# vlongle/pixie

Measured on AMD Instinct MI355X. Metric: voxels/s (128^3 U-Net fwd) + MPM particle-steps/s, higher is better.
Workload: dtype f32 (operands split fp16 hi+lo, 3 f16 MFMAs/product, fp32 accumulate); 1 GPU; 128^3x64 feature grid -> SegmentationUNet+RegressionUNet forward (+argmax/one-hot combine), 1 scene per GPU per step; grid=128, feature_channels=64, parallelism=scene-parallel x1, executor=c+hip_graph

## Files before the change

### include/pixie_hip.h

```cpp
#ifndef PIXIE_HIP_H
#define PIXIE_HIP_H

#include <stdint.h>

#ifdef __cplusplus
extern "C" {
#endif

const char* pixie_last_error(void);
const char* pixie_build_arch(void);

typedef struct pixie_mpm pixie_mpm;

int pixie_mpm_create(pixie_mpm** out, int n_particles, int n_grid, double grid_lim);
int pixie_mpm_destroy(pixie_mpm* h);
int pixie_mpm_regrid(pixie_mpm* h, int n_grid, double grid_lim, void* stream);

int pixie_mpm_set_field(pixie_mpm* h, const char* name, const void* d_src, int64_t count, void* stream);
int pixie_mpm_get_field(pixie_mpm* h, const char* name, void* d_dst, int64_t count, void* stream);
int pixie_mpm_fill_field(pixie_mpm* h, const char* name, double value, void* stream);

int pixie_mpm_set_scalar(pixie_mpm* h, const char* key, double value);
int pixie_mpm_get_scalar(pixie_mpm* h, const char* key, double* value);

// ... 133 lines not shown

int pixie_combine_class_ids(const int32_t* d_seg_pred, int num_classes, const float* d_cont, int64_t spatial, float* d_combined,
                            void* stream);

typedef struct pixie_unet pixie_unet;
typedef struct pixie_unet_config {
    int32_t feature_channels, cond_dim, model_channels, num_res_blocks;
    int32_t n_channel_mult; int32_t channel_mult[8];
    int32_t n_attention_resolutions; int32_t attention_resolutions[8];
    int32_t grid_size;
    int32_t out_channels;
    int32_t precision;
} pixie_unet_config;

int pixie_unet_create(pixie_unet** out, const pixie_unet_config* cfg);
int pixie_unet_destroy(pixie_unet* h);
int pixie_unet_param_count(const pixie_unet* h);
int pixie_unet_param_info(const pixie_unet* h, int index, const char** key, int64_t* numel, int32_t* ndim, int64_t shape[5]);
int pixie_unet_set_param(pixie_unet* h, const char* key, const float* d_values, int64_t numel);
int64_t pixie_unet_workspace_bytes(pixie_unet* h, int d, int hh, int w);
int pixie_unet_forward(pixie_unet* h, const float* d_feat, const float* d_proj0, int d, int hh, int w, float* d_out,
                       void* d_workspace, int64_t workspace_bytes, void* stream);
int pixie_unet_set_option(pixie_unet* h, const char* key, int value);

typedef struct pixie_field_desc {
    const float* d_pred;
    const uint8_t* d_mask;
    const float* d_axis_x; const float* d_axis_y; const float* d_axis_z;
    int32_t n_classes, d, h, w;
    double min_spacing;
    double density_min, density_max, E_min, E_max, nu_min, nu_max;
} pixie_field_desc;
int pixie_field_to_particles(const pixie_field_desc* field, const float* d_pos, int n, int k, double nn_distance_threshold,
                             int weighted, int default_material, int default_part_label, float* d_density, float* d_E,
                             float* d_nu, int32_t* d_material, int32_t* d_part_label, float* d_conf, float* d_nearest,
                             void* d_scratch, void* stream);

int pixie_unscale_prediction(const float* d_pred, int channels, int64_t spatial, double density_min, double density_max,
                             double E_min, double E_max, double nu_min, double nu_max, float* d_out, void* stream);
int64_t pixie_field_points_scratch_bytes(const pixie_field_desc* field);
int pixie_field_points(const pixie_field_desc* field, int64_t capacity, float* d_xyz , float* d_density, float* d_E,
                       float* d_nu, int32_t* d_material, float* d_conf, int64_t* d_count, void* d_scratch, void* stream);

int pixie_dbscan_roots(const float* d_pos_sorted, const int32_t* d_orig_index, const int32_t* d_cell_start, int n, int nx, int ny, int nz,
                       const double lo[3], double cell_size, double eps, int min_samples, int32_t* d_core_scratch,
                       int32_t* d_parent_scratch, int32_t* d_root, void* stream);
// ... 51 lines not shown
```

### pixie_amd/_lib.py

```python
from __future__ import annotations

import ctypes as C
import os

_HERE = os.path.dirname(os.path.abspath(__file__))
LIB_PATH = os.path.join(_HERE, "libpixie_hip.so")
DIAG_LIB_PATH = os.path.join(_HERE, "libpixie_hip_diag.so")


class PixieHipError(RuntimeError):
    pass


class BCDesc(C.Structure):
    _fields_ = [("type", C.c_int32), ("surface_type", C.c_int32), ("reset", C.c_int32), ("pad_", C.c_int32),
                ("point", C.c_double * 3), ("size", C.c_double * 3), ("velocity", C.c_double * 3),
                ("normal", C.c_double * 3), ("start_time", C.c_double), ("end_time", C.c_double),
                ("friction", C.c_double)]


class PModDesc(C.Structure):
    _fields_ = [("type", C.c_int32), ("pad_", C.c_int32),
                ("point", C.c_double * 3), ("size", C.c_double * 3), ("force", C.c_double * 3),
                ("velocity", C.c_double * 3), ("normal", C.c_double * 3), ("h1", C.c_double * 3),
# ... 100 lines not shown
    "pixie_conv_subpixel_bytes": (_I64, [_I, _I]),
    "pixie_conv_pack_weights_subpixel": (_I, [_VP, _VP, _I, _I, _VP]),
    "pixie_conv3d_forward": (_I, [C.POINTER(ConvDesc), _VP]),
    "pixie_conv_stats_floats": (_I64, [C.POINTER(ConvDesc)]),
    "pixie_conv_workspace_bytes": (_I64, [C.POINTER(ConvDesc)]),
    "pixie_stats_finalize": (_I, [_VP, C.POINTER(ConvDesc), _VP, _VP]),
    "pixie_stats_norm_finalize": (_I, [_VP, C.POINTER(ConvDesc), _VP, _VP, C.POINTER(ConvDesc), _VP, _I, _I64, _I, _I, _D, _VP, _VP, _VP, _VP, _VP]),
    "pixie_channel_stats": (_I, [_VP, _I, _I64, _VP, _VP, _VP]),
    "pixie_tensor_amax": (_I, [_VP, _I64, _VP, _VP]),
    "pixie_channel_sums": (_I, [_VP, _I, _I64, _VP, _VP]),
    "pixie_norm_finalize": (_I, [_VP, _I, _I64, _I, _I, _D, _VP, _VP, _VP, _VP, _VP]),
    "pixie_attention_forward": (_I, [_VP, _VP, _I, _I, _VP]),
    "pixie_channel_affine": (_I, [_VP, _VP, _VP, _VP, _I, _I64, _VP]),
    "pixie_projector_conv0": (_I, [_VP, _I64, _I, _I, C.POINTER(_VP), C.POINTER(_VP), C.POINTER(_VP), _I, _VP]),
    "pixie_conv_skip_foldable": (_I, [C.POINTER(ConvDesc)]),
    "pixie_unet_create": (_I, [C.POINTER(_VP), C.POINTER(UNetConfigC)]),
    "pixie_unet_destroy": (_I, [_VP]),
    "pixie_unet_param_count": (_I, [_VP]),
    "pixie_unet_param_info": (_I, [_VP, _I, C.POINTER(_S), C.POINTER(_I64), C.POINTER(C.c_int32), C.POINTER(_I64)]),
    "pixie_unet_set_param": (_I, [_VP, _S, _VP, _I64]),
    "pixie_unet_workspace_bytes": (_I64, [_VP, _I, _I, _I]),
    "pixie_unet_set_option": (_I, [_VP, _S, _I]),
    "pixie_unet_forward": (_I, [_VP, _VP, _VP, _I, _I, _I, _VP, _VP, _I64, _VP]),
    "pixie_combine_class_ids": (_I, [_VP, _I, _VP, _I64, _VP, _VP]),
    "pixie_combine_predictions": (_I, [_VP, _I, _VP, _I64, _VP, _VP, _VP]),
    "pixie_voxel_grid_to_ncdhw": (_I, [_VP, _I, _I, _I, _I, _VP, _VP]),
    "pixie_unscale_prediction": (_I, [_VP, _I, _I64, _D, _D, _D, _D, _D, _D, _VP, _VP]),
    "pixie_field_points_scratch_bytes": (_I64, [C.POINTER(FieldDesc)]),
    "pixie_field_points": (_I, [C.POINTER(FieldDesc), _I64, _VP, _VP, _VP, _VP, _VP, _VP, _VP, _VP, _VP]),
    "pixie_fill_densify": (_I, [_VP, _VP, _VP, _I, _I, _D, _VP, _VP, _VP]),
    "pixie_fill_dense_cells": (_I, [_VP, _VP, _I, _D, _D, _I, _VP, _I64, _VP, C.c_uint32, _VP]),
    "pixie_fill_internal_cells": (_I, [_VP, _VP, _I, _D, _I, _I, _I, _D, _VP, _I64, _VP, C.c_uint32, _VP]),
    "pixie_particle_volume": (_I, [_VP, _I, _I, _D, _VP, _VP, _VP]),
    "pixie_nearest_particle": (_I, [_VP, _I, _VP, _I, _VP, _VP]),
    "pixie_dbscan_roots": (_I, [_VP, _VP, _VP, _I, _I, _I, _I, C.POINTER(_D), _D, _D, _I, _VP, _VP, _VP, _VP]),
    "pixie_raster_workspace_bytes": (_I64, [_I, _I, _I, _I64]),
    "pixie_raster_forward": (_I, [C.POINTER(RasterDesc), C.POINTER(_I64), _VP]),
    "pixie_sh_to_rgb": (_I, [_VP, _I64, _I, _I, _VP, C.POINTER(C.c_float), _VP, _I64, _VP, _VP]),
    "pixie_field_to_particles": (_I, [C.POINTER(FieldDesc), _VP, _I, _I, _D, _I, _I, _I, _VP, _VP, _VP, _VP, _VP, _VP, _VP, _VP, _VP]),
}

DIAG_SIGNATURES = {
    "pixie_mpm_phase": (_I, [_VP, _I, _D, _VP]),
    "pixie_mpm_kernel_times": (_I, [_VP, C.POINTER(_D), C.POINTER(_D), C.POINTER(_I64)]),
    "pixie_conv_kernel_variant": (C.c_int, [C.POINTER(ConvDesc), C.POINTER(C.c_int)]),
    "pixie_conv_tile_geometry": (C.c_int, [C.POINTER(ConvDesc), C.POINTER(C.c_int32)]),
# ... 41 lines not shown
```

### pixie_amd/csrc/unet_exec.hip

```cpp
#include <hip/hip_runtime.h>

#include <algorithm>
#include <cmath>
#include <cstdlib>
#include <cstring>
#include <map>
#include <memory>
#include <stdexcept>
#include <string>
#include <tuple>
#include <unordered_map>
#include <vector>

#include "../../include/pixie_hip.h"
#include "common.h"

namespace pixie {
int channel_stats_prezeroed(const float* d_x, int channels, int64_t spatial, double* d_sums, uint32_t* d_amax, hipStream_t st);
int norm_finalize_cat(const double* d_sums0, int c0, const double* d_sums1, int c1, int64_t spatial, int mode, int groups, double eps,
                      const float* d_weight, const float* d_bias, float* d_a, float* d_b, hipStream_t st);
namespace {

enum { ACT_NONE = 0, ACT_LEAKY = 1, ACT_SILU = 2 };
enum Kind { CONV_IN, RES, DOWN, ATTN, UP };
// ... 161 lines not shown
            used_[off] = bytes;
            if (off + bytes > peak) peak = off + bytes;
            return off;
        }
        fail("pixie_unet_forward: the workspace is too small (%lld bytes; ask pixie_unet_workspace_bytes for this grid size)", (long long)capacity);
    }
    void release(int64_t off) {
        auto u = used_.find(off);
        if (u == used_.end()) return;
        int64_t size = u->second;
        used_.erase(u);
        auto next = free_.lower_bound(off);
        if (next != free_.end() && off + size == next->first) { size += next->second; next = free_.erase(next); }
        if (next != free_.begin()) {
            auto prev = std::prev(next);
            if (prev->first + prev->second == off) { prev->second += size; return; }
        }
        free_[off] = size;
    }
    template <class T> T* ptr(int64_t off) const { return reinterpret_cast<T*>(base + off); }
};

struct Exec;
struct Tens {
    Exec* ex = nullptr;
    float* p = nullptr;
    int64_t off = -1;
    int c = 0, d = 0, h = 0, w = 0;
    int64_t sums_off = -1;
    bool has_sums = false;
    double* sums = nullptr;
    int64_t partials_off = -1;
    pixie_conv_desc pdesc;
    uint32_t* slot = nullptr;
    int64_t spatial() const { return (int64_t)d * h * w; }
    ~Tens();
};
using TP = std::shared_ptr<Tens>;

struct Packed { void* d = nullptr; uint64_t version = ~0ull; };
struct Sized { int64_t bytes; int slots; int64_t zsum_doubles; };
struct Bound { float wmax = 0, bmax = 0; uint64_t wver = ~0ull, bver = ~0ull; };

}
}

using namespace pixie;

struct pixie_unet {
    Cfg cfg;
    Plan plan;
    std::vector<Param> params;
    std::unordered_map<std::string, int> index;
    std::unordered_map<std::string, Packed> packed32, packed16;
    std::unordered_map<std::string, Bound> bounds;
    uint32_t* d_bound_slots = nullptr;
    std::vector<uint32_t> h_bound_slots;
    std::map<std::tuple<int, int, int, bool>, Sized> sized;
    bool fuse_stats = true, split_k = true, fold_skip = true, subpixel = true;
    bool split_stats = true;
    struct Replay { const float* feat; const float* proj0; float* out; void* ws; int d; uint64_t epoch; hipGraph_t graph; hipGraphExec_t exec; };
    bool use_graph = false;
    uint64_t epoch = 0;
    std::vector<Replay> replays;
    static constexpr size_t kMaxReplays = 4;
    void drop_replay(size_t i) {
        (void)hipGraphExecDestroy(replays[i].exec);
        (void)hipGraphDestroy(replays[i].graph);
        replays.erase(replays.begin() + (long)i);
    }

    const Param& param(const std::string& key) const {
        auto it = index.find(key);
        if (it == index.end()) fail("pixie_unet: no parameter named '%s'", key.c_str());
        return params[it->second];
    }
};

namespace pixie {
namespace {

struct Exec {
    pixie_unet* net = nullptr;
    Arena arena;
    bool dry = false;
    void* stream = nullptr;
    uint32_t* slots = nullptr;
    int slot_next = 0, slot_cap = 0;
// ... 49 lines not shown
        if (dry) return nullptr;
        Packed& e = net->packed32[key];
        if (e.version != p.version) {
            const int cout = (int)p.shape[0], cin = (int)p.shape[1], k = (int)p.shape[2];
            int64_t taps = 1;
            for (size_t i = 2; i < p.shape.size(); ++i) taps *= p.shape[i];
            const int64_t nb = taps * cin * pixie_conv_cout_padded(cout) * (int64_t)sizeof(float);
            if (!e.d && hipMalloc(&e.d, (size_t)nb) != hipSuccess) fail("pixie_unet: hipMalloc of %lld bytes failed", (long long)nb);
            if (!p.d) fail("pixie_unet_forward: parameter '%s.weight' was never set", key.c_str());
            ok(pixie_conv_pack_weights(p.d, static_cast<float*>(e.d), cout, cin, k, stream), "pixie_conv_pack_weights");
            e.version = p.version;
        }
        return static_cast<const float*>(e.d);
    }
    float norm_bound(const std::string& key, int64_t count) {
        if (dry) return 1.0f;
        const Bound& b = net->bounds[key];
        return (float)(std::sqrt((double)count) * (double)b.wmax + (double)b.bmax + 1e-30);
    }

    void stats(const TP& t) {
        if (t->has_sums || t->partials_off >= 0) return;
        t->has_sums = true;
        if (!dry && zsum_next + 2 * t->c > zsum_cap) fail("pixie_unet_forward: out of statistics space (internal sizing error)");
        t->sums = dry ? nullptr : zsums + zsum_next;
        zsum_next += 2 * t->c;
        t->slot = new_slot();
        if (!dry) ok(channel_stats_prezeroed(t->p, t->c, t->spatial(), t->sums, t->slot, as_stream(stream)), "pixie_channel_stats");
    }
    struct AB { std::shared_ptr<Scratch> mem; float* a; float* b; };
    AB norm_finalize(const std::vector<TP>& parts, int64_t spatial, int mode, int groups, const float* w, const float* b) {
        for (auto& t : parts) stats(t);
        const Tens* t0 = parts[0].get();
        const Tens* t1 = parts.size() > 1 ? parts[1].get() : nullptr;
        const int c0 = t0->c, c1 = t1 ? t1->c : 0, c = c0 + c1;
        AB r;
        const int cpad = (c + 63) / 64 * 64;
        r.mem = std::make_shared<Scratch>(this, (int64_t)(cpad + c) * sizeof(float));
        r.a = r.mem->as<float>();
        r.b = r.a + cpad;
        const bool p0 = t0->partials_off >= 0, p1 = t1 && t1->partials_off >= 0;
        if (p0 || p1) {
            pixie_conv_desc d0 = t0->pdesc;
            if (!p0) { std::memset(&d0, 0, sizeof d0); d0.c_out = c0; }
            if (!dry) ok(pixie_stats_norm_finalize(p0 ? arena.ptr<float>(t0->partials_off) : nullptr, &d0, t0->sums,
                                                   p1 ? arena.ptr<float>(t1->partials_off) : nullptr, p1 ? &t1->pdesc : nullptr, t1 ? t1->sums : nullptr,
// ... 140 lines not shown
        const int64_t spatial = x->spatial();
        AB pro = norm_finalize({x}, spatial, 1, 32, P(p + ".norm.weight"), P(p + ".norm.bias"));
        ConvOpt o; o.pro = &pro; o.bound = norm_bound(p + ".norm", spatial * (c / 32));
        TP qkv = conv({x}, p + ".qkv", 3 * c, 1, o);
        TP att = make(c, x->d, x->h, x->w);
        if (!dry) ok(pixie_attention_forward(qkv->p, att->p, c, (int)spatial, stream), "pixie_attention_forward");
        qkv.reset();
        ConvOpt o2; o2.residual = x;
        return conv({att}, p + ".proj_out", c, 1, o2);
    }
    TP block(const Blk& b, const std::vector<TP>& parts, const Tens* up_to) {
        if (b.kind == RES) return res(b, parts);
        const TP& x = parts[0];
        if (b.kind == ATTN) return attn(b, x);
        if (b.kind == DOWN) { ConvOpt o; o.stride = 2; return conv({x}, b.prefix + ".op", b.cout, 3, o); }
        if (b.kind == UP) {
            ConvOpt o; o.upsample = true;
            if (up_to) { o.out_d = up_to->d; o.out_h = up_to->h; o.out_w = up_to->w; }
            return conv({x}, b.prefix + ".conv", b.cout, 3, o);
        }
        fail("pixie_unet: unexpected block kind");
    }

    TP forward(const float* d_feat, const float* d_proj0, int D, int H, int W, float* d_out) {
        const Cfg& c = net->cfg;
        const int64_t spatial = (int64_t)D * H * W;
        TP x;
        AB pro_in; const AB* pro_in_p = nullptr;
        int act_in = ACT_NONE; float bound_in = 0.0f;
        if (c.has_projector()) {
            const std::string q = "projector.net.";
            const int hid = c.projector_hidden();
            if (!hid) {
                const int g = std::max(c.cond_dim / 2, 1);
                x = conv({external(d_feat, c.feature_channels, D, H, W)}, q + "0", c.cond_dim, 1, ConvOpt{});
                pro_in = norm_finalize({x}, spatial, 1, g, P(q + "1.weight"), P(q + "1.bias"));
                act_in = ACT_SILU;
                bound_in = norm_bound(q + "1", spatial * (c.cond_dim / g));
            } else {
                if (d_proj0) x = external(d_proj0, hid, D, H, W);
                else x = conv({external(d_feat, c.feature_channels, D, H, W)}, q + "0", hid, 1, ConvOpt{});
                AB pro = norm_finalize({x}, spatial, 1, 32, P(q + "1.weight"), P(q + "1.bias"));
                ConvOpt o; o.pro = &pro; o.act = ACT_SILU; o.bound = norm_bound(q + "1", spatial * (hid / 32));
                x = conv({x}, q + "3", hid, 3, o);
                AB pro2 = norm_finalize({x}, spatial, 1, 32, P(q + "4.weight"), P(q + "4.bias"));
                ConvOpt o2; o2.pro = &pro2; o2.act = ACT_SILU; o2.bound = norm_bound(q + "4", spatial * (hid / 32));
                x = conv({x}, q + "6", c.cond_dim, 1, o2);
                pro_in = norm_finalize({x}, spatial, 1, 32, P(q + "7.weight"), P(q + "7.bias"));
                bound_in = norm_bound(q + "7", spatial * std::max(c.cond_dim / 32, 1));
            }
            pro_in_p = &pro_in;
        } else {
            x = external(d_feat, c.feature_channels, D, H, W);
        }
        const Plan& plan = net->plan;
        std::vector<TP> hs;
        const Blk& first = plan.in_blocks[0][0];
        ConvOpt of; of.pro = pro_in_p; of.act = act_in; of.bound = bound_in;
        TP h = conv({x}, first.prefix, first.cout, 3, of);
        x.reset();
        pro_in = AB{};
        hs.push_back(h);
        for (size_t i = 1; i < plan.in_blocks.size(); ++i) {
            for (const Blk& b : plan.in_blocks[i]) h = block(b, {h}, nullptr);
            hs.push_back(h);
        }
        for (const Blk& b : plan.middle) h = block(b, {h}, nullptr);
        for (auto& seq : plan.out_blocks) {
            TP skip = hs.back(); hs.pop_back();
            if (skip->d != h->d || skip->h != h->h || skip->w != h->w) fail("pixie_unet_forward: skip tensor and decoder tensor differ in size");
            std::vector<TP> parts{h, skip};
            h.reset(); skip.reset();
            for (const Blk& b : seq) {
                TP nh = block(b, parts, (b.kind == UP && !hs.empty()) ? hs.back().get() : nullptr);
                parts.clear();
                parts.push_back(nh);
            }
            h = parts[0];
        }
        AB pro = norm_finalize({h}, h->spatial(), 0, 1, nullptr, nullptr);
        ConvOpt oo; oo.pro = &pro; oo.affine_store = "unet.out.0"; oo.act = ACT_LEAKY; oo.bound = norm_bound("unet.out.0", h->spatial());
        oo.out_ptr = d_out;
        return conv({h}, "unet.out.2", c.out_channels, 3, oo);
    }
};

Tens::~Tens() {
    if (!ex) return;
    if (off >= 0) ex->arena.release(off);
    if (sums_off >= 0) ex->arena.release(sums_off);
    if (partials_off >= 0) ex->arena.release(partials_off);
}

void refresh_bounds(pixie_unet* net, void* stream) {
    std::vector<std::pair<std::string, int>> todo;
    int n_norm = 0;
    for (const Param& p : net->params) {
        if (!p.norm || p.key.size() < 7 || p.key.compare(p.key.size() - 7, 7, ".weight") != 0) continue;
        const std::string key = p.key.substr(0, p.key.size() - 7);
        const Param& pb = net->param(key + ".bias");
        Bound& b = net->bounds[key];
        if (b.wver != p.version || b.bver != pb.version) todo.push_back({key, 2 * n_norm});
        ++n_norm;
    }
    if (todo.empty()) return;
    const size_t bytes = (size_t)2 * n_norm * sizeof(uint32_t);
// ... 25 lines not shown
    if (i < n16) p[i] = make_uint4(0u, 0u, 0u, 0u);
}

constexpr int64_t kSlotAlign = 256;
int64_t slot_region_bytes(int n_slots) { return ((int64_t)n_slots * 4 + kSlotAlign - 1) / kSlotAlign * kSlotAlign; }
int64_t zsum_region_bytes(int64_t n_doubles) { return (n_doubles * 8 + kSlotAlign - 1) / kSlotAlign * kSlotAlign; }

Sized size_pass(pixie_unet* net, int D, int H, int W, bool from_proj0) {
    auto key = std::make_tuple(D, H, W, from_proj0);
    auto it = net->sized.find(key);
    if (it != net->sized.end()) return it->second;
    Exec ex;
    ex.net = net; ex.dry = true; ex.stream = nullptr;
    ex.arena.reset(reinterpret_cast<char*>(0x10000000), (int64_t)1 << 50);
    {
        const float* fake = reinterpret_cast<const float*>(0x100);
        TP out = ex.forward(from_proj0 ? nullptr : fake, from_proj0 ? fake : nullptr, D, H, W, reinterpret_cast<float*>(0x100));
    }
    Sized r{ex.arena.peak + slot_region_bytes(ex.slot_next) + zsum_region_bytes(ex.zsum_next), ex.slot_next, ex.zsum_next};
    net->sized[key] = r;
    return r;
}

template <class F> int guarded(F f) {
    try { return f(); }
    catch (const std::exception& e) { return set_error("%s", e.what()); }
}

}
}

extern "C" int pixie_unet_create(pixie_unet** out, const pixie_unet_config* c) {
    PX_REQUIRE(out && c, "pixie_unet_create: null argument");
    PX_REQUIRE(c->n_channel_mult >= 1 && c->n_channel_mult <= 8 && c->n_attention_resolutions >= 0 && c->n_attention_resolutions <= 8,
               "pixie_unet_create: channel_mult needs 1..8 entries, attention_resolutions 0..8");
    PX_REQUIRE(c->feature_channels > 0 && c->cond_dim > 0 && c->model_channels > 0 && c->num_res_blocks > 0 && c->grid_size > 0 && c->out_channels > 0,
               "pixie_unet_create: non-positive size");
    PX_REQUIRE(c->precision == 0 || c->precision == 1, "pixie_unet_create: precision is 0 (f16x3) or 1 (exact fp32)");
    return guarded([&] {
        std::unique_ptr<pixie_unet> n(new pixie_unet);
        n->cfg.feature_channels = c->feature_channels; n->cfg.cond_dim = c->cond_dim; n->cfg.model_channels = c->model_channels;
        n->cfg.num_res_blocks = c->num_res_blocks; n->cfg.grid_size = c->grid_size; n->cfg.out_channels = c->out_channels;
        n->cfg.precision = c->precision;
        n->cfg.mult.assign(c->channel_mult, c->channel_mult + c->n_channel_mult);
        n->cfg.attn.assign(c->attention_resolutions, c->attention_resolutions + c->n_attention_resolutions);
        n->plan = build_plan(n->cfg);
        n->params = param_table(n->cfg, n->plan);
        for (size_t i = 0; i < n->params.size(); ++i) n->index[n->params[i].key] = (int)i;
        const char* fs = getenv("PIXIE_FUSE_STATS"); n->fuse_stats = !(fs && fs[0] == '0');
        const char* sk = getenv("PIXIE_CONV_SPLIT_K"); n->split_k = !(sk && sk[0] == '0');
        const char* fk = getenv("PIXIE_FOLD_SKIP"); n->fold_skip = !(fk && fk[0] == '0');
        const char* ss = getenv("PIXIE_SPLIT_STATS"); n->split_stats = !(ss && ss[0] == '0');
        const char* sx = getenv("PIXIE_CONV_SUBPIXEL"); n->subpixel = !(sx && sx[0] == '0');
        *out = n.release();
        return 0;
    });
}

extern "C" int pixie_unet_destroy(pixie_unet* h) {
    if (!h) return 0;
    for (auto& kv : h->packed16) if (kv.second.d) (void)hipFree(kv.second.d);
    for (auto& kv : h->packed32) if (kv.second.d) (void)hipFree(kv.second.d);
    if (h->d_bound_slots) (void)hipFree(h->d_bound_slots);
    while (!h->replays.empty()) h->drop_replay(0);
    delete h;
    return 0;
}

extern "C" int pixie_unet_param_count(const pixie_unet* h) { return h ? (int)h->params.size() : 0; }

extern "C" int pixie_unet_param_info(const pixie_unet* h, int i, const char** key, int64_t* numel, int32_t* ndim, int64_t shape[5]) {
    PX_REQUIRE(h && i >= 0 && i < (int)h->params.size(), "pixie_unet_param_info: index out of range");
    const Param& p = h->params[i];
    if (key) *key = p.key.c_str();
    if (numel) *numel = p.numel;
    if (ndim) *ndim = (int32_t)p.shape.size();
    if (shape) for (size_t k = 0; k < p.shape.size() && k < 5; ++k) shape[k] = p.shape[k];
    return 0;
}

extern "C" int pixie_unet_set_param(pixie_unet* h, const char* key, const float* d_values, int64_t numel) {
    PX_REQUIRE(h && key && d_values, "pixie_unet_set_param: null argument");
    auto it = h->index.find(key);
    PX_REQUIRE(it != h->index.end(), "pixie_unet_set_param: unexpected key '%s' (the reference's load_state_dict(strict=True) raises here too)", key);
    Param& p = h->params[it->second];
    PX_REQUIRE(numel == p.numel, "pixie_unet_set_param: '%s' has %lld elements, got %lld", key, (long long)p.numel, (long long)numel);
    p.d = d_values;
// ... 6 lines not shown
    if (!h || d <= 0 || hh <= 0 || w <= 0) { set_error("pixie_unet_workspace_bytes: bad argument"); return -1; }
    int64_t bytes = -1;
    const int rc = guarded([&] {
        bytes = size_pass(h, d, hh, w, false).bytes;
        if (h->cfg.projector_hidden() > 0) bytes = std::max(bytes, size_pass(h, d, hh, w, true).bytes);
        return 0;
    });
    return rc == 0 ? bytes : -1;
}

extern "C" int pixie_unet_forward(pixie_unet* h, const float* d_feat, const float* d_proj0, int d, int hh, int w, float* d_out,
                                  void* d_workspace, int64_t workspace_bytes, void* stream) {
    PX_REQUIRE(h && d_out && d_workspace && (d_feat || d_proj0), "pixie_unet_forward: null argument");
    PX_REQUIRE(d == h->cfg.grid_size && hh == d && w == d,
               "pixie_unet_forward: the network was built for a %d^3 grid (its LayerNorm parameters have that shape), got %d x %d x %d", h->cfg.grid_size, d, hh, w);
    PX_REQUIRE(!d_proj0 || h->cfg.projector_hidden() > 0, "pixie_unet_forward: d_proj0 needs the hidden-128 projector (feature_channels > cond_dim)");
    PX_REQUIRE(d_feat || (d_proj0 && h->cfg.has_projector()), "pixie_unet_forward: d_feat is null");
    return guarded([&] {
        const auto sized = size_pass(h, d, hh, w, d_proj0 != nullptr);
        if (workspace_bytes < sized.bytes)
            fail("pixie_unet_forward: workspace of %lld bytes, this grid needs %lld (pixie_unet_workspace_bytes)", (long long)workspace_bytes, (long long)sized.bytes);
        auto launch_all = [&] {
            Exec ex;
            ex.net = h; ex.dry = false; ex.stream = stream;
            const int64_t slot_bytes = slot_region_bytes(sized.slots), head_bytes = slot_bytes + zsum_region_bytes(sized.zsum_doubles);
            ex.slots = static_cast<uint32_t*>(d_workspace);
            ex.slot_cap = sized.slots;
            ex.zsums = reinterpret_cast<double*>(static_cast<char*>(d_workspace) + slot_bytes);
            ex.zsum_cap = sized.zsum_doubles;
            hipLaunchKernelGGL(zero_head_kernel, dim3((unsigned)((head_bytes / 16 + 255) / 256)), dim3(256), 0, as_stream(stream),
                               static_cast<uint4*>(d_workspace), head_bytes / 16);
            if (hipGetLastError() != hipSuccess) fail("pixie_unet_forward: clearing the workspace head failed");
            ex.arena.reset(static_cast<char*>(d_workspace) + head_bytes, workspace_bytes - head_bytes);
            TP out = ex.forward(d_feat, d_proj0, d, hh, w, d_out);
        };
        if (h->use_graph) {
            for (size_t i = 0; i < h->replays.size(); ++i) {
                const pixie_unet::Replay& r = h->replays[i];
                if (r.feat != d_feat || r.proj0 != d_proj0 || r.out != d_out || r.ws != d_workspace || r.d != d) continue;
                if (r.epoch != h->epoch) { h->drop_replay(i); break; }
                if (hipGraphLaunch(r.exec, as_stream(stream)) != hipSuccess) fail("pixie_unet_forward: hipGraphLaunch failed: %s", hipGetErrorString(hipGetLastError()));
                if (i + 1 != h->replays.size()) std::rotate(h->replays.begin() + (long)i, h->replays.begin() + (long)i + 1, h->replays.end());
                return 0;
            }
        }
        if (h->use_graph && as_stream(stream) == nullptr)
            fail("pixie_unet_forward: option \"graph\" needs a non-default stream (the legacy stream cannot be captured); pass a created stream or set graph = 0");
        refresh_bounds(h, stream);
        launch_all();
        if (h->use_graph) {
            hipStream_t st = as_stream(stream);
            if (hipStreamBeginCapture(st, hipStreamCaptureModeThreadLocal) != hipSuccess)
                fail("pixie_unet_forward: cannot capture on this stream (graph replay needs a non-default stream): %s", hipGetErrorString(hipGetLastError()));
            hipGraph_t graph = nullptr;
            try { launch_all(); }
            catch (...) { (void)hipStreamEndCapture(st, &graph); if (graph) (void)hipGraphDestroy(graph); throw; }
            if (hipStreamEndCapture(st, &graph) != hipSuccess || !graph) fail("pixie_unet_forward: hipStreamEndCapture failed: %s", hipGetErrorString(hipGetLastError()));
            hipGraphExec_t exec = nullptr;
            if (hipGraphInstantiate(&exec, graph, nullptr, nullptr, 0) != hipSuccess) { (void)hipGraphDestroy(graph); fail("pixie_unet_forward: hipGraphInstantiate failed"); }
            if (h->replays.size() >= pixie_unet::kMaxReplays) h->drop_replay(0);
            h->replays.push_back(pixie_unet::Replay{d_feat, d_proj0, d_out, d_workspace, d, h->epoch, graph, exec});
        }
        return 0;
    });
}

extern "C" int pixie_unet_set_option(pixie_unet* h, const char* key, int value) {
    PX_REQUIRE(h && key, "pixie_unet_set_option: null argument");
    const std::string k(key);
    if (k == "graph") {
        h->use_graph = value != 0;
        if (!h->use_graph) while (!h->replays.empty()) h->drop_replay(0);
        return 0;
    }
    return set_error("pixie_unet_set_option: unknown key '%s' (known: graph)", key);
}
```

### pixie_amd/unet.py

```python
from __future__ import annotations

import ctypes as C
import math
import os
import warnings
import weakref
from typing import Dict, List, Optional, Sequence, Tuple

import torch
import torch.nn as nn

from . import _lib
from ._lib import ConvDesc, check
from .unet_plan import Block, UNetConfig, UNetPlan, build_plan, param_shapes, is_norm_key

ACT_NONE, ACT_LEAKY, ACT_SILU = 0, 1, 2
DEFAULT_PRECISION = os.environ.get("PIXIE_CONV_PRECISION", "f16x3")
_ZERO_INIT_SUFFIXES = (".out_layers.3.weight", ".out_layers.3.bias", ".proj_out.weight", ".proj_out.bias",
                       "unet.out.2.weight", "unet.out.2.bias")


def _ptr(t: Optional[torch.Tensor]):
    return C.c_void_p(t.data_ptr()) if t is not None else C.c_void_p(0)

# ... 667 lines not shown
        graph, static_in, static_out = ent
        if static_in is not None:
            static_in.copy_(src)
        graph.replay()
        return static_out.clone()


class SegmentationUNet(_PixieUNet):

    def __init__(self, feature_channels: int, cond_dim: int, model_channels: int, num_res_blocks: int,
                 channel_mult: Tuple[int, ...], attention_resolutions: Tuple[int, ...], grid_size: int, num_classes: int):
        super().__init__(UNetConfig(feature_channels, cond_dim, model_channels, num_res_blocks, tuple(channel_mult),
                                    tuple(attention_resolutions), grid_size, num_classes))


class RegressionUNet(_PixieUNet):

    def __init__(self, feature_channels: int, cond_dim: int, model_channels: int, num_res_blocks: int,
                 channel_mult: Tuple[int, ...], attention_resolutions: Tuple[int, ...], grid_size: int, out_channels: int = 3):
        super().__init__(UNetConfig(feature_channels, cond_dim, model_channels, num_res_blocks, tuple(channel_mult),
                                    tuple(attention_resolutions), grid_size, out_channels))


@torch.no_grad()
def predict_material_field_from_voxel_grid(seg_network: "SegmentationUNet", cont_network: "RegressionUNet", grid_dhwc_f16: torch.Tensor,
                                           dual_stream: Optional[bool] = None):
    dev = next(seg_network.parameters()).device
    g = grid_dhwc_f16
    if g.dim() != 4 or g.dtype != torch.float16 or g.device != dev or dev.type != "cuda":
        raise ValueError("expected a (D, H, W, C) float16 tensor on the networks' HIP device")
    nets = (seg_network, cont_network)
    for net in nets:
        if net.cfg.projector_hidden is None or net.cfg.feature_channels != g.shape[3] or net.conv_precision != "f16x3":
            raise ValueError("the fused grid path needs the hidden-128 projector, matching feature_channels and conv_precision 'f16x3'")
        net._prepare(dev)
    ops = seg_network._runner.ops
    q = "projector.net.0"
    packed = [(net._runner._w16(q), net._runner._b(q)) for net in nets]
    x_seg, x_cont = ops.projector_conv0(g, packed, seg_network.cfg.projector_hidden)
    if dual_stream is None:
        dual_stream = _dual_stream_default(seg_network, cont_network, int(g.shape[0]) * int(g.shape[1]) * int(g.shape[2]))

    def fwd(net, p0):
        return net._forward_graphed(None, p0) if net.use_graph else net._forward_one(None, proj0=p0)

    if dual_stream:
        cur = torch.cuda.current_stream()
        s1, s2 = _side_streams(dev)
        s1.wait_stream(cur); s2.wait_stream(cur)
        with torch.cuda.stream(s1):
            seg_logits = fwd(seg_network, x_seg)[None]
        with torch.cuda.stream(s2):
            cont_pred = fwd(cont_network, x_cont)[None]
        x_seg.record_stream(s1); x_cont.record_stream(s2)
        cur.wait_stream(s1); cur.wait_stream(s2)
        seg_logits.record_stream(cur); cont_pred.record_stream(cur)
    else:
        seg_logits = fwd(seg_network, x_seg)[None]
        cont_pred = fwd(cont_network, x_cont)[None]
    combined, seg_pred = ops.combine(seg_logits[0].contiguous(), cont_pred[0].contiguous())
    return combined[None], seg_pred[None], seg_logits, cont_pred


_SIDE_STREAMS: Dict[str, Tuple[torch.cuda.Stream, torch.cuda.Stream]] = {}


def _dual_stream_default(seg_network, cont_network, voxels: int) -> bool:
    env = os.environ.get("PIXIE_DUAL_STREAM")
    if env is not None:
        return env == "1"
    return not (seg_network.use_graph and cont_network.use_graph and voxels >= 128 ** 3)


def _side_streams(device):
    key = str(device)
    if key not in _SIDE_STREAMS:
        _SIDE_STREAMS[key] = (torch.cuda.Stream(device), torch.cuda.Stream(device))
    return _SIDE_STREAMS[key]


@torch.no_grad()
def predict_material_field(seg_network: SegmentationUNet, cont_network: RegressionUNet, feat_grid: torch.Tensor,
                           dual_stream: Optional[bool] = None):
    if feat_grid.is_cuda and feat_grid.device.index != torch.cuda.current_device():
        with torch.cuda.device(feat_grid.device):
            return predict_material_field(seg_network, cont_network, feat_grid, dual_stream)
    if dual_stream is None:
        dual_stream = _dual_stream_default(seg_network, cont_network, int(feat_grid[0, 0].numel()))
    if dual_stream and feat_grid.is_cuda:
        cur = torch.cuda.current_stream()
        s1, s2 = _side_streams(feat_grid.device)
        s1.wait_stream(cur); s2.wait_stream(cur)
        with torch.cuda.stream(s1):
            seg_logits = seg_network(feat_grid)
        with torch.cuda.stream(s2):
            cont_pred = cont_network(feat_grid)
        feat_grid.record_stream(s1); feat_grid.record_stream(s2)
        cur.wait_stream(s1); cur.wait_stream(s2)
        seg_logits.record_stream(cur); cont_pred.record_stream(cur)
    else:
        seg_logits = seg_network(feat_grid)
        cont_pred = cont_network(feat_grid)
    ops = seg_network._runner.ops
    combined, seg_pred = [], []
    for n in range(feat_grid.shape[0]):
        cmb, am = ops.combine(seg_logits[n].contiguous(), cont_pred[n].contiguous())
        combined.append(cmb)
        seg_pred.append(am)
    return torch.stack(combined), torch.stack(seg_pred), seg_logits, cont_pred
```

Measured before the change: 24.09 million voxels/s.

## Run segmentation and regression U-Nets as one paired graph with shared input stats

Adds a paired forward that records both U-Net passes into a single HIP graph over one shared workspace. When both nets read the same feature input, its channel statistics are computed once and reused. An optional staggered schedule runs each net's coarse levels on a side stream so they overlap with the other net's work. The aim is to cut launch and graph overhead and duplicated statistics work when the two nets would otherwise run sequentially. In exchange it adds workspace, output clones or copies, more code paths, and replay caching keyed on pointers.

```diff
diff --git a/include/pixie_hip.h b/include/pixie_hip.h
--- a/include/pixie_hip.h
+++ b/include/pixie_hip.h
@@ -179,6 +179,9 @@
 int pixie_unet_forward(pixie_unet* h, const float* d_feat, const float* d_proj0, int d, int hh, int w, float* d_out,
                        void* d_workspace, int64_t workspace_bytes, void* stream);
 int pixie_unet_set_option(pixie_unet* h, const char* key, int value);
+int64_t pixie_unet_pair_workspace_bytes(pixie_unet* a, pixie_unet* b, int d, int hh, int w, int64_t layout[6]);
+int pixie_unet_pair_forward(pixie_unet* a, pixie_unet* b, const float* d_feat, const float* d_proj0_a, const float* d_proj0_b,
+                            int d, int hh, int w, float* d_out_a, float* d_out_b, void* d_workspace, int64_t workspace_bytes, void* stream);
 
 typedef struct pixie_field_desc {
     const float* d_pred;
diff --git a/pixie_amd/_lib.py b/pixie_amd/_lib.py
--- a/pixie_amd/_lib.py
+++ b/pixie_amd/_lib.py
@@ -146,6 +146,8 @@
     "pixie_unet_workspace_bytes": (_I64, [_VP, _I, _I, _I]),
     "pixie_unet_set_option": (_I, [_VP, _S, _I]),
     "pixie_unet_forward": (_I, [_VP, _VP, _VP, _I, _I, _I, _VP, _VP, _I64, _VP]),
+    "pixie_unet_pair_workspace_bytes": (_I64, [_VP, _VP, _I, _I, _I, C.POINTER(_I64)]),
+    "pixie_unet_pair_forward": (_I, [_VP, _VP, _VP, _VP, _VP, _I, _I, _I, _VP, _VP, _VP, _I64, _VP]),
     "pixie_combine_class_ids": (_I, [_VP, _I, _VP, _I64, _VP, _VP]),
     "pixie_combine_predictions": (_I, [_VP, _I, _VP, _I64, _VP, _VP, _VP]),
     "pixie_voxel_grid_to_ncdhw": (_I, [_VP, _I, _I, _I, _I, _VP, _VP]),
diff --git a/pixie_amd/csrc/unet_exec.hip b/pixie_amd/csrc/unet_exec.hip
--- a/pixie_amd/csrc/unet_exec.hip
+++ b/pixie_amd/csrc/unet_exec.hip
@@ -207,6 +207,7 @@
 };
 
 struct Exec;
+struct SharedStats { double* sums = nullptr; uint32_t* slot = nullptr; bool done = false; };
 struct Tens {
     Exec* ex = nullptr;
     float* p = nullptr;
@@ -218,6 +219,7 @@
     int64_t partials_off = -1;
     pixie_conv_desc pdesc;
     uint32_t* slot = nullptr;
+    struct SharedStats* shared = nullptr;
     int64_t spatial() const { return (int64_t)d * h * w; }
     ~Tens();
 };
@@ -249,6 +251,19 @@
     uint64_t epoch = 0;
     std::vector<Replay> replays;
     static constexpr size_t kMaxReplays = 4;
+    struct PairReplay { uint64_t other; const float* feat; const float* proj0[2]; float* out[2]; void* ws; int d; int schedule; uint64_t epoch[2];
+                        hipGraph_t graph; hipGraphExec_t exec; };
+    uint64_t uid = 0;
+    bool pair_graph = false;
+    int pair_schedule = 0;
+    std::vector<PairReplay> pair_replays;
+    hipStream_t pair_side = nullptr;
+    hipEvent_t pair_events[4] = {nullptr, nullptr, nullptr, nullptr};
+    void drop_pair_replay(size_t i) {
+        (void)hipGraphExecDestroy(pair_replays[i].exec);
+        (void)hipGraphDestroy(pair_replays[i].graph);
+        pair_replays.erase(pair_replays.begin() + (long)i);
+    }
     void drop_replay(size_t i) {
         (void)hipGraphExecDestroy(replays[i].exec);
         (void)hipGraphDestroy(replays[i].graph);
@@ -344,6 +359,12 @@
     void stats(const TP& t) {
         if (t->has_sums || t->partials_off >= 0) return;
         t->has_sums = true;
+        if (t->shared) {
+            t->sums = t->shared->sums; t->slot = t->shared->slot;
+            if (!t->shared->done) ok(channel_stats_prezeroed(t->p, t->c, t->spatial(), t->sums, t->slot, as_stream(stream)), "pixie_channel_stats");
+            t->shared->done = true;
+            return;
+        }
         if (!dry && zsum_next + 2 * t->c > zsum_cap) fail("pixie_unet_forward: out of statistics space (internal sizing error)");
         t->sums = dry ? nullptr : zsums + zsum_next;
         zsum_next += 2 * t->c;
@@ -530,24 +551,27 @@
         fail("pixie_unet: unexpected block kind");
     }
 
-    TP forward(const float* d_feat, const float* d_proj0, int D, int H, int W, float* d_out) {
+    struct Walk { std::vector<TP> hs; TP h; size_t in_next = 1; size_t coarse_end = 0; } walk;
+
+    void encode_full(const float* d_feat, const float* d_proj0, int D, int H, int W, SharedStats* shared) {
         const Cfg& c = net->cfg;
         const int64_t spatial = (int64_t)D * H * W;
         TP x;
         AB pro_in; const AB* pro_in_p = nullptr;
         int act_in = ACT_NONE; float bound_in = 0.0f;
+        auto input = [&] { TP t = external(d_feat, c.feature_channels, D, H, W); t->shared = shared; return t; };
         if (c.has_projector()) {
             const std::string q = "projector.net.";
             const int hid = c.projector_hidden();
             if (!hid) {
                 const int g = std::max(c.cond_dim / 2, 1);
-                x = conv({external(d_feat, c.feature_channels, D, H, W)}, q + "0", c.cond_dim, 1, ConvOpt{});
+                x = conv({input()}, q + "0", c.cond_dim, 1, ConvOpt{});
                 pro_in = norm_finalize({x}, spatial, 1, g, P(q + "1.weight"), P(q + "1.bias"));
                 act_in = ACT_SILU;
                 bound_in = norm_bound(q + "1", spatial * (c.cond_dim / g));
             } else {
                 if (d_proj0) x = external(d_proj0, hid, D, H, W);
-                else x = conv({external(d_feat, c.feature_channels, D, H, W)}, q + "0", hid, 1, ConvOpt{});
+                else x = conv({input()}, q + "0", hid, 1, ConvOpt{});
                 AB pro = norm_finalize({x}, spatial, 1, 32, P(q + "1.weight"), P(q + "1.bias"));
                 ConvOpt o; o.pro = &pro; o.act = ACT_SILU; o.bound = norm_bound(q + "1", spatial * (hid / 32));
                 x = conv({x}, q + "3", hid, 3, o);
@@ -559,37 +583,62 @@
             }
             pro_in_p = &pro_in;
         } else {
-            x = external(d_feat, c.feature_channels, D, H, W);
+            x = input();
         }
         const Plan& plan = net->plan;
-        std::vector<TP> hs;
         const Blk& first = plan.in_blocks[0][0];
         ConvOpt of; of.pro = pro_in_p; of.act = act_in; of.bound = bound_in;
-        TP h = conv({x}, first.prefix, first.cout, 3, of);
+        walk = Walk{};
+        walk.h = conv({x}, first.prefix, first.cout, 3, of);
         x.reset();
         pro_in = AB{};
-        hs.push_back(h);
-        for (size_t i = 1; i < plan.in_blocks.size(); ++i) {
-            for (const Blk& b : plan.in_blocks[i]) h = block(b, {h}, nullptr);
-            hs.push_back(h);
-        }
-        for (const Blk& b : plan.middle) h = block(b, {h}, nullptr);
-        for (auto& seq : plan.out_blocks) {
-            TP skip = hs.back(); hs.pop_back();
-            if (skip->d != h->d || skip->h != h->h || skip->w != h->w) fail("pixie_unet_forward: skip tensor and decoder tensor differ in size");
-            std::vector<TP> parts{h, skip};
-            h.reset(); skip.reset();
-            for (const Blk& b : seq) {
-                TP nh = block(b, parts, (b.kind == UP && !hs.empty()) ? hs.back().get() : nullptr);
-                parts.clear();
-                parts.push_back(nh);
-            }
-            h = parts[0];
-        }
+        walk.hs.push_back(walk.h);
+        for (size_t k = 0; k < plan.out_blocks.size(); ++k)
+            for (const Blk& b : plan.out_blocks[k]) if (b.kind == UP) walk.coarse_end = k + 1;
+        bool down = false;
+        while (walk.in_next < plan.in_blocks.size() && !down) down = in_block(walk.in_next++);
+    }
+    bool in_block(size_t i) {
+        bool down = false;
+        for (const Blk& b : net->plan.in_blocks[i]) { walk.h = block(b, {walk.h}, nullptr); down = down || b.kind == DOWN; }
+        walk.hs.push_back(walk.h);
+        return down;
+    }
+    void out_block(size_t k) {
+        std::vector<TP>& hs = walk.hs;
+        TP& h = walk.h;
+        TP skip = hs.back(); hs.pop_back();
+        if (skip->d != h->d || skip->h != h->h || skip->w != h->w) fail("pixie_unet_forward: skip tensor and decoder tensor differ in size");
+        std::vector<TP> parts{h, skip};
+        h.reset(); skip.reset();
+        for (const Blk& b : net->plan.out_blocks[k]) {
+            TP nh = block(b, parts, (b.kind == UP && !hs.empty()) ? hs.back().get() : nullptr);
+            parts.clear();
+            parts.push_back(nh);
+        }
+        h = parts[0];
+    }
+    void middle() { for (const Blk& b : net->plan.middle) walk.h = block(b, {walk.h}, nullptr); }
+    void coarse() {
+        while (walk.in_next < net->plan.in_blocks.size()) in_block(walk.in_next++);
+        if (!walk.coarse_end) return;
+        middle();
+        for (size_t k = 0; k < walk.coarse_end; ++k) out_block(k);
+    }
+    TP decode_full(float* d_out) {
+        if (!walk.coarse_end) middle();
+        for (size_t k = walk.coarse_end; k < net->plan.out_blocks.size(); ++k) out_block(k);
+        TP h = walk.h;
+        walk = Walk{};
         AB pro = norm_finalize({h}, h->spatial(), 0, 1, nullptr, nullptr);
         ConvOpt oo; oo.pro = &pro; oo.affine_store = "unet.out.0"; oo.act = ACT_LEAKY; oo.bound = norm_bound("unet.out.0", h->spatial());
         oo.out_ptr = d_out;
-        return conv({h}, "unet.out.2", c.out_channels, 3, oo);
+        return conv({h}, "unet.out.2", net->cfg.out_channels, 3, oo);
+    }
+    TP forward(const float* d_feat, const float* d_proj0, int D, int H, int W, float* d_out) {
+        encode_full(d_feat, d_proj0, D, H, W, nullptr);
+        coarse();
+        return decode_full(d_out);
     }
 };
 
@@ -661,6 +710,46 @@
     return r;
 }
 
+void begin_pass(Exec& ex, pixie_unet* net, char* ws, int64_t ws_bytes, const Sized& sized, int64_t lead_bytes, void* stream) {
+    ex.net = net; ex.dry = false; ex.stream = stream;
+    const int64_t slot_bytes = slot_region_bytes(sized.slots), head_bytes = slot_bytes + zsum_region_bytes(sized.zsum_doubles);
+    ex.slots = reinterpret_cast<uint32_t*>(ws);
+    ex.slot_cap = sized.slots;
+    ex.zsums = reinterpret_cast<double*>(ws + slot_bytes);
+    ex.zsum_cap = sized.zsum_doubles;
+    const int64_t n16 = (lead_bytes + head_bytes) / 16;
+    hipLaunchKernelGGL(zero_head_kernel, dim3((unsigned)((n16 + 255) / 256)), dim3(256), 0, as_stream(stream), reinterpret_cast<uint4*>(ws - lead_bytes), n16);
+    if (hipGetLastError() != hipSuccess) fail("pixie_unet_forward: clearing the workspace head failed");
+    ex.arena.reset(ws + head_bytes, ws_bytes - head_bytes);
+}
+
+template <class F> void record_graph(hipStream_t st, F&& launch_all, hipGraph_t* graph, hipGraphExec_t* exec) {
+    if (hipStreamBeginCapture(st, hipStreamCaptureModeThreadLocal) != hipSuccess)
+        fail("pixie_unet_forward: cannot capture on this stream (graph replay needs a non-default stream): %s", hipGetErrorString(hipGetLastError()));
+    try { launch_all(); }
+    catch (...) { (void)hipStreamEndCapture(st, graph); if (*graph) (void)hipGraphDestroy(*graph); throw; }
+    if (hipStreamEndCapture(st, graph) != hipSuccess || !*graph) fail("pixie_unet_forward: hipStreamEndCapture failed: %s", hipGetErrorString(hipGetLastError()));
+    if (hipGraphInstantiate(exec, *graph, nullptr, nullptr, 0) != hipSuccess) { (void)hipGraphDestroy(*graph); fail("pixie_unet_forward: hipGraphInstantiate failed"); }
+}
+
+struct PairLayout { int64_t amax_off, sums_off, part_off[2], part_bytes[2], total; };
+PairLayout pair_layout(pixie_unet* a, pixie_unet* b, int d, int hh, int w) {
+    pixie_unet* nets[2] = {a, b};
+    PairLayout l;
+    l.amax_off = 0;
+    l.sums_off = kSlotAlign;
+    int64_t off = l.sums_off + zsum_region_bytes(2 * (int64_t)a->cfg.feature_channels);
+    for (int i = 0; i < 2; ++i) {
+        int64_t bytes = size_pass(nets[i], d, hh, w, false).bytes;
+        if (nets[i]->cfg.projector_hidden() > 0) bytes = std::max(bytes, size_pass(nets[i], d, hh, w, true).bytes);
+        l.part_off[i] = off;
+        l.part_bytes[i] = (bytes + kSlotAlign - 1) / kSlotAlign * kSlotAlign;
+        off += l.part_bytes[i];
+    }
+    l.total = off;
+    return l;
+}
+
 template <class F> int guarded(F f) {
     try { return f(); }
     catch (const std::exception& e) { return set_error("%s", e.what()); }
@@ -678,6 +767,8 @@
     PX_REQUIRE(c->precision == 0 || c->precision == 1, "pixie_unet_create: precision is 0 (f16x3) or 1 (exact fp32)");
     return guarded([&] {
         std::unique_ptr<pixie_unet> n(new pixie_unet);
+        static uint64_t next_uid = 0;
+        n->uid = ++next_uid;
         n->cfg.feature_channels = c->feature_channels; n->cfg.cond_dim = c->cond_dim; n->cfg.model_channels = c->model_channels;
         n->cfg.num_res_blocks = c->num_res_blocks; n->cfg.grid_size = c->grid_size; n->cfg.out_channels = c->out_channels;
         n->cfg.precision = c->precision;
@@ -702,6 +793,9 @@
     for (auto& kv : h->packed32) if (kv.second.d) (void)hipFree(kv.second.d);
     if (h->d_bound_slots) (void)hipFree(h->d_bound_slots);
     while (!h->replays.empty()) h->drop_replay(0);
+    while (!h->pair_replays.empty()) h->drop_pair_replay(0);
+    for (hipEvent_t e : h->pair_events) if (e) (void)hipEventDestroy(e);
+    if (h->pair_side) (void)hipStreamDestroy(h->pair_side);
     delete h;
     return 0;
 }
@@ -754,16 +848,7 @@
             fail("pixie_unet_forward: workspace of %lld bytes, this grid needs %lld (pixie_unet_workspace_bytes)", (long long)workspace_bytes, (long long)sized.bytes);
         auto launch_all = [&] {
             Exec ex;
-            ex.net = h; ex.dry = false; ex.stream = stream;
-            const int64_t slot_bytes = slot_region_bytes(sized.slots), head_bytes = slot_bytes + zsum_region_bytes(sized.zsum_doubles);
-            ex.slots = static_cast<uint32_t*>(d_workspace);
-            ex.slot_cap = sized.slots;
-            ex.zsums = reinterpret_cast<double*>(static_cast<char*>(d_workspace) + slot_bytes);
-            ex.zsum_cap = sized.zsum_doubles;
-            hipLaunchKernelGGL(zero_head_kernel, dim3((unsigned)((head_bytes / 16 + 255) / 256)), dim3(256), 0, as_stream(stream),
-                               static_cast<uint4*>(d_workspace), head_bytes / 16);
-            if (hipGetLastError() != hipSuccess) fail("pixie_unet_forward: clearing the workspace head failed");
-            ex.arena.reset(static_cast<char*>(d_workspace) + head_bytes, workspace_bytes - head_bytes);
+            begin_pass(ex, h, static_cast<char*>(d_workspace), workspace_bytes, sized, 0, stream);
             TP out = ex.forward(d_feat, d_proj0, d, hh, w, d_out);
         };
         if (h->use_graph) {
@@ -781,15 +866,9 @@
         refresh_bounds(h, stream);
         launch_all();
         if (h->use_graph) {
-            hipStream_t st = as_stream(stream);
-            if (hipStreamBeginCapture(st, hipStreamCaptureModeThreadLocal) != hipSuccess)
-                fail("pixie_unet_forward: cannot capture on this stream (graph replay needs a non-default stream): %s", hipGetErrorString(hipGetLastError()));
             hipGraph_t graph = nullptr;
-            try { launch_all(); }
-            catch (...) { (void)hipStreamEndCapture(st, &graph); if (graph) (void)hipGraphDestroy(graph); throw; }
-            if (hipStreamEndCapture(st, &graph) != hipSuccess || !graph) fail("pixie_unet_forward: hipStreamEndCapture failed: %s", hipGetErrorString(hipGetLastError()));
             hipGraphExec_t exec = nullptr;
-            if (hipGraphInstantiate(&exec, graph, nullptr, nullptr, 0) != hipSuccess) { (void)hipGraphDestroy(graph); fail("pixie_unet_forward: hipGraphInstantiate failed"); }
+            record_graph(as_stream(stream), launch_all, &graph, &exec);
             if (h->replays.size() >= pixie_unet::kMaxReplays) h->drop_replay(0);
             h->replays.push_back(pixie_unet::Replay{d_feat, d_proj0, d_out, d_workspace, d, h->epoch, graph, exec});
         }
@@ -805,5 +884,117 @@
         if (!h->use_graph) while (!h->replays.empty()) h->drop_replay(0);
         return 0;
     }
-    return set_error("pixie_unet_set_option: unknown key '%s' (known: graph)", key);
-}
+    if (k == "pair_graph") {
+        h->pair_graph = value != 0;
+        if (!h->pair_graph) while (!h->pair_replays.empty()) h->drop_pair_replay(0);
+        return 0;
+    }
+    if (k == "pair_schedule") {
+        PX_REQUIRE(value == 0 || value == 1, "pixie_unet_set_option: pair_schedule is 0 (back to back) or 1 (staggered)");
+        h->pair_schedule = value;
+        return 0;
+    }
+    return set_error("pixie_unet_set_option: unknown key '%s' (known: graph, pair_graph, pair_schedule)", key);
+}
+
+extern "C" int64_t pixie_unet_pair_workspace_bytes(pixie_unet* a, pixie_unet* b, int d, int hh, int w, int64_t layout[6]) {
+    if (!a || !b || a == b || d <= 0 || hh <= 0 || w <= 0) { set_error("pixie_unet_pair_workspace_bytes: bad argument"); return -1; }
+    int64_t bytes = -1;
+    const int rc = guarded([&] {
+        const PairLayout l = pair_layout(a, b, d, hh, w);
+        if (layout) { layout[0] = l.amax_off; layout[1] = l.sums_off; layout[2] = l.part_off[0]; layout[3] = l.part_bytes[0]; layout[4] = l.part_off[1]; layout[5] = l.part_bytes[1]; }
+        bytes = l.total;
+        return 0;
+    });
+    return rc == 0 ? bytes : -1;
+}
+
+extern "C" int pixie_unet_pair_forward(pixie_unet* a, pixie_unet* b, const float* d_feat, const float* d_proj0_a, const float* d_proj0_b,
+                                       int d, int hh, int w, float* d_out_a, float* d_out_b, void* d_workspace, int64_t workspace_bytes, void* stream) {
+    PX_REQUIRE(a && b && a != b && d_out_a && d_out_b && d_out_a != d_out_b && d_workspace, "pixie_unet_pair_forward: null argument, or one handle or output given twice");
+    PX_REQUIRE((d_feat && !d_proj0_a && !d_proj0_b) || (d_proj0_a && d_proj0_b), "pixie_unet_pair_forward: give d_feat, or d_proj0 of both networks");
+    pixie_unet* nets[2] = {a, b};
+    const float* proj0[2] = {d_proj0_a, d_proj0_b};
+    float* outs[2] = {d_out_a, d_out_b};
+    for (pixie_unet* n : nets) {
+        PX_REQUIRE(d == n->cfg.grid_size && hh == d && w == d,
+                   "pixie_unet_pair_forward: the network was built for a %d^3 grid (its LayerNorm parameters have that shape), got %d x %d x %d", n->cfg.grid_size, d, hh, w);
+        PX_REQUIRE(d_feat || n->cfg.projector_hidden() > 0, "pixie_unet_pair_forward: d_proj0 needs the hidden-128 projector (feature_channels > cond_dim)");
+    }
+    PX_REQUIRE(a->cfg.feature_channels == b->cfg.feature_channels, "pixie_unet_pair_forward: the two networks read one grid, but expect %d and %d feature channels",
+               a->cfg.feature_channels, b->cfg.feature_channels);
+    return guarded([&] {
+        const PairLayout lay = pair_layout(a, b, d, hh, w);
+        if (workspace_bytes < lay.total)
+            fail("pixie_unet_pair_forward: workspace of %lld bytes, this pair needs %lld (pixie_unet_pair_workspace_bytes)", (long long)workspace_bytes, (long long)lay.total);
+        const int schedule = a->pair_schedule;
+        const Sized sized[2] = {size_pass(a, d, hh, w, d_proj0_a != nullptr), size_pass(b, d, hh, w, d_proj0_b != nullptr)};
+        char* ws = static_cast<char*>(d_workspace);
+        hipStream_t main_st = as_stream(stream);
+        auto launch_all = [&] {
+            Exec ex[2];
+            SharedStats shared;
+            shared.slot = reinterpret_cast<uint32_t*>(ws + lay.amax_off);
+            shared.sums = reinterpret_cast<double*>(ws + lay.sums_off);
+            hipEvent_t* ev = a->pair_events;
+            auto record = [&](hipEvent_t e, hipStream_t st) {
+                if (hipEventRecord(e, st) != hipSuccess) fail("pixie_unet_pair_forward: hipEventRecord failed: %s", hipGetErrorString(hipGetLastError()));
+            };
+            auto wait = [&](hipStream_t st, hipEvent_t e) {
+                if (hipStreamWaitEvent(st, e, 0) != hipSuccess) fail("pixie_unet_pair_forward: hipStreamWaitEvent failed: %s", hipGetErrorString(hipGetLastError()));
+            };
+            auto E = [&](int i) {
+                begin_pass(ex[i], nets[i], ws + lay.part_off[i], lay.part_bytes[i], sized[i], i == 0 ? lay.part_off[0] : 0, stream);
+                ex[i].encode_full(d_feat, proj0[i], d, hh, w, d_feat ? &shared : nullptr);
+            };
+            if (schedule == 0) {
+                for (int i = 0; i < 2; ++i) { E(i); ex[i].coarse(); TP out = ex[i].decode_full(outs[i]); }
+                return;
+            }
+            hipStream_t side = a->pair_side;
+            E(0);
+            record(ev[0], main_st); wait(side, ev[0]);
+            ex[0].stream = side; ex[0].coarse();
+            record(ev[1], side);
+            E(1);
+            record(ev[2], main_st); wait(side, ev[2]);
+            ex[1].stream = side; ex[1].coarse();
+            record(ev[3], side);
+            wait(main_st, ev[1]);
+            ex[0].stream = stream; { TP out = ex[0].decode_full(outs[0]); }
+            wait(main_st, ev[3]);
+            ex[1].stream = stream; { TP out = ex[1].decode_full(outs[1]); }
+        };
+        const uint64_t epochs[2] = {a->epoch, b->epoch};
+        if (a->pair_graph) {
+            for (size_t i = 0; i < a->pair_replays.size(); ++i) {
+                const pixie_unet::PairReplay& r = a->pair_replays[i];
+                if (r.other != b->uid || r.feat != d_feat || r.proj0[0] != d_proj0_a || r.proj0[1] != d_proj0_b || r.out[0] != d_out_a || r.out[1] != d_out_b ||
+                    r.ws != d_workspace || r.d != d || r.schedule != schedule) continue;
+                if (r.epoch[0] != epochs[0] || r.epoch[1] != epochs[1]) { a->drop_pair_replay(i); break; }
+                if (hipGraphLaunch(r.exec, main_st) != hipSuccess) fail("pixie_unet_pair_forward: hipGraphLaunch failed: %s", hipGetErrorString(hipGetLastError()));
+                if (i + 1 != a->pair_replays.size()) std::rotate(a->pair_replays.begin() + (long)i, a->pair_replays.begin() + (long)i + 1, a->pair_replays.end());
+                return 0;
+            }
+            if (main_st == nullptr)
+                fail("pixie_unet_pair_forward: option \"pair_graph\" needs a non-default stream (the legacy stream cannot be captured); pass a created stream or set pair_graph = 0");
+        }
+        if (schedule == 1 && !a->pair_side) {
+            if (hipStreamCreateWithFlags(&a->pair_side, hipStreamNonBlocking) != hipSuccess) fail("pixie_unet_pair_forward: hipStreamCreate failed");
+            for (hipEvent_t& e : a->pair_events)
+                if (hipEventCreateWithFlags(&e, hipEventDisableTiming) != hipSuccess) fail("pixie_unet_pair_forward: hipEventCreate failed");
+        }
+        refresh_bounds(a, stream);
+        refresh_bounds(b, stream);
+        launch_all();
+        if (a->pair_graph) {
+            hipGraph_t graph = nullptr;
+            hipGraphExec_t exec = nullptr;
+            record_graph(main_st, launch_all, &graph, &exec);
+            if (a->pair_replays.size() >= pixie_unet::kMaxReplays) a->drop_pair_replay(0);
+            a->pair_replays.push_back(pixie_unet::PairReplay{b->uid, d_feat, {d_proj0_a, d_proj0_b}, {d_out_a, d_out_b}, d_workspace, d, schedule,
+                                                             {epochs[0], epochs[1]}, graph, exec});
+        }
+        return 0;
+    });
+}
diff --git a/pixie_amd/unet.py b/pixie_amd/unet.py
--- a/pixie_amd/unet.py
+++ b/pixie_amd/unet.py
@@ -713,6 +713,79 @@
                                     tuple(attention_resolutions), grid_size, out_channels))
 
 
+class _PairRunner:
+
+    def __init__(self, seg: "_PixieUNet", cont: "_PixieUNet", dev: torch.device, dhw: Tuple[int, int, int]):
+        self.lib = _lib.load()
+        self.key = (id(cont), id(seg._handle), id(cont._handle), dev, dhw)
+        self.handles = (seg._handle, cont._handle)
+        a, b = (h._h for h in self.handles)
+        n = int(self.lib.pixie_unet_pair_workspace_bytes(a, b, *dhw, None))
+        if n < 0:
+            raise _lib.PixieHipError(self.lib.pixie_last_error().decode())
+        self.nbytes = n
+        self.workspace = torch.empty(n, device=dev, dtype=torch.uint8)
+        self.outs = tuple(torch.empty((net.cfg.out_channels,) + dhw, device=dev, dtype=torch.float32) for net in (seg, cont))
+        self.stream = torch.cuda.Stream(dev)
+        self.in_place_ptr: Optional[int] = None
+        self.private: Dict[Tuple, torch.Tensor] = {}
+        check(self.lib.pixie_unet_set_option(a, b"pair_graph", 1), "pixie_unet_set_option")
+
+    def run(self, feat: Optional[torch.Tensor], proj0: Optional[Tuple[torch.Tensor, torch.Tensor]], schedule: int):
+        srcs = (feat,) if proj0 is None else tuple(proj0)
+        if proj0 is None and self.in_place_ptr in (None, feat.data_ptr()):
+            self.in_place_ptr = feat.data_ptr()
+            ins = srcs
+        else:
+            ins = []
+            for i, t in enumerate(srcs):
+                buf = self.private.get((i, tuple(t.shape)))
+                if buf is None:
+                    buf = self.private[(i, tuple(t.shape))] = torch.empty_like(t)
+                buf.copy_(t)
+                ins.append(buf)
+        a, b = (h._h for h in self.handles)
+        check(self.lib.pixie_unet_set_option(a, b"pair_schedule", schedule), "pixie_unet_set_option")
+        d, h, w = (int(v) for v in ins[0].shape[1:])
+        cur = torch.cuda.current_stream()
+        self.stream.wait_stream(cur)
+        with torch.cuda.stream(self.stream):
+            check(self.lib.pixie_unet_pair_forward(a, b, _ptr(ins[0]) if proj0 is None else None,
+                                                   _ptr(ins[0]) if proj0 is not None else None, _ptr(ins[1]) if proj0 is not None else None,
+                                                   d, h, w, _ptr(self.outs[0]), _ptr(self.outs[1]), _ptr(self.workspace), self.nbytes,
+                                                   _lib.current_stream_ptr()), "pixie_unet_pair_forward")
+        for t in ins:
+            t.record_stream(self.stream)
+        cur.wait_stream(self.stream)
+        return self.outs
+
+
+def _pair_schedule_default() -> int:
+    env = os.environ.get("PIXIE_PAIR_SCHEDULE")
+    if env is not None:
+        return 1 if env == "1" else 0
+    return _PAIR_SCHEDULE_DEFAULT
+
+
+_PAIR_SCHEDULE_DEFAULT = 0
+
+
+def _pair_runner(seg_network, cont_network, dev: torch.device, dhw, dual_stream: bool) -> Optional[_PairRunner]:
+    nets = (seg_network, cont_network)
+    if dual_stream or dev.type != "cuda" or any(n.executor != "c" or not n.use_graph or n.conv_precision != "f16x3" for n in nets):
+        return None
+    if next(cont_network.parameters()).device != dev or seg_network is cont_network:
+        return None
+    for net in nets:
+        net._prepare(dev)
+    key = (id(cont_network), id(seg_network._handle), id(cont_network._handle), dev, tuple(dhw))
+    pair = seg_network.__dict__.get("_pair")
+    if pair is None or pair.key != key:
+        pair = _PairRunner(seg_network, cont_network, dev, tuple(dhw))
+        seg_network.__dict__["_pair"] = pair
+    return pair
+
+
 @torch.no_grad()
 def predict_material_field_from_voxel_grid(seg_network: "SegmentationUNet", cont_network: "RegressionUNet", grid_dhwc_f16: torch.Tensor,
                                            dual_stream: Optional[bool] = None):
@@ -735,7 +808,10 @@
     def fwd(net, p0):
         return net._forward_graphed(None, p0) if net.use_graph else net._forward_one(None, proj0=p0)
 
-    if dual_stream:
+    pair = _pair_runner(seg_network, cont_network, dev, tuple(int(v) for v in g.shape[:3]), dual_stream)
+    if pair is not None:
+        seg_logits, cont_pred = (t.clone()[None] for t in pair.run(None, (x_seg, x_cont), _pair_schedule_default()))
+    elif dual_stream:
         cur = torch.cuda.current_stream()
         s1, s2 = _side_streams(dev)
         s1.wait_stream(cur); s2.wait_stream(cur)
@@ -778,7 +854,20 @@
             return predict_material_field(seg_network, cont_network, feat_grid, dual_stream)
     if dual_stream is None:
         dual_stream = _dual_stream_default(seg_network, cont_network, int(feat_grid[0, 0].numel()))
-    if dual_stream and feat_grid.is_cuda:
+    pair = None
+    if feat_grid.is_cuda and feat_grid.dim() == 5 and feat_grid.shape[1] == seg_network.cfg.feature_channels == cont_network.cfg.feature_channels \
+            and next(seg_network.parameters()).device == feat_grid.device:
+        pair = _pair_runner(seg_network, cont_network, feat_grid.device, tuple(int(v) for v in feat_grid.shape[2:]), dual_stream)
+    if pair is not None:
+        x = feat_grid.detach().to(torch.float32).contiguous()
+        n_samples = x.shape[0]
+        seg_logits = torch.empty((n_samples,) + tuple(pair.outs[0].shape), device=x.device, dtype=torch.float32)
+        cont_pred = torch.empty((n_samples,) + tuple(pair.outs[1].shape), device=x.device, dtype=torch.float32)
+        for n in range(n_samples):
+            lg, cp = pair.run(x[n], None, _pair_schedule_default())
+            seg_logits[n].copy_(lg)
+            cont_pred[n].copy_(cp)
+    elif dual_stream and feat_grid.is_cuda:
         cur = torch.cuda.current_stream()
         s1, s2 = _side_streams(feat_grid.device)
         s1.wait_stream(cur); s2.wait_stream(cur)
```

Measured after the change: 24.12 million voxels/s (median of 4 runs). Within noise of the previous version (+0.2%).
